# GiantAI/pixtrack

Measured on AMD Instinct MI355X. Metric: tracked frames/sec at 640x480 (full NeRF render + UNet + LM loop), higher is better.
Workload: dtype fp16 storage / fp32 accumulate (UNet, NeRF MLPs); fp32 (LM)

## Files before the change

include/pixtrack_hip.h:

```cpp
#ifndef PIXTRACK_HIP_H
#define PIXTRACK_HIP_H

#include <stdint.h>

#ifdef __cplusplus
extern "C" {
#endif

#define PXT_OK 0
#define PXT_E_ARG -1
#define PXT_E_HIP -2
#define PXT_E_TIMEOUT -3
#define PXT_E_STATE -4

#define PXT_MAX_LEVELS 8
#define PXT_LM_LOG_STRIDE 20

int pxt_version(void);
const char* pxt_last_error(void);
int pxt_device_cus(int* n_cus_host);

typedef struct {
  const float* fmap;
  const float* fref;
// ... 133 lines not shown
  int32_t width, height, spp;
  int32_t mode;
} pxt_ngp_view;

int pxt_ngp_render(pxt_ngp* ctx, const pxt_ngp_view* view_host, float* out_rgba,
                   uint64_t* stats ,
                   void* stream);

int pxt_ngp_render_both(pxt_ngp* ctx, const pxt_ngp_view* view_host, float* out_rgba, float* out_depth_rgba,
                        uint64_t* stats, void* stream);

int pxt_ngp_render_both_from_pose(pxt_ngp* ctx, const pxt_ngp_view* view_host, const float* pose12,
                                  const double* conv27_host, float* cam_out13, float* out_rgba,
                                  float* out_depth_rgba, uint64_t* stats, void* stream);

typedef struct {
  float* rgba;
  float* depth_rgba;
  uint8_t* rgb_u8;
  uint8_t* depth_nz;
} pxt_ngp_outputs;
int pxt_ngp_render_frame(pxt_ngp* ctx, const pxt_ngp_view* view_host, int32_t mode, int32_t camera_from_slot,
                         const pxt_ngp_outputs* out, uint64_t* stats, void* stream);
float* pxt_ngp_camera_slot(pxt_ngp* ctx);

#define PXT_NGP_MAX_BATCH 16
int64_t pxt_ngp_batch_workspace_bytes(int32_t n_renders);
int pxt_ngp_render_frame_batch(pxt_ngp* const* ctxs, const pxt_ngp_view* views_host, int32_t n_renders,
                               const int32_t* modes, int32_t camera_from_slot, const pxt_ngp_outputs* outs_host,
                               uint64_t* const* stats, void* batch_workspace, void* stream);

int pxt_ngp_create_shared(pxt_ngp* src, pxt_ngp** out_ctx);

int pxt_ngp_timing_enable(pxt_ngp* ctx, int32_t every_nth);
int pxt_ngp_timing_read(pxt_ngp* ctx, float* total_ms_host, int32_t* n_launches_host);

int pxt_ngp_query(pxt_ngp* ctx, const float* pos, const float* dir, int32_t n, float* out, void* stream);

int pxt_depth_mask(const float* depth_rgba, int32_t H, int32_t W, int32_t n_erode,
                   int32_t n_dilate, uint8_t* mask_out, uint8_t* tmp, void* stream);
int pxt_depth_mask_plane(const uint8_t* depth_nz, int32_t H, int32_t W, int32_t n_erode, int32_t n_dilate,
                         uint8_t* mask_out, uint8_t* tmp, void* stream);
int pxt_rgba_to_u8(const float* rgba, int32_t H, int32_t W, float alpha_thresh, uint8_t* rgb_out,
                   void* stream);
int pxt_resize_linear(const float* src, int32_t H, int32_t W, int32_t C, float* dst, int32_t Ho,
                      int32_t Wo, void* stream);

int pxt_resize_activity(const uint8_t* mask, const uint8_t* image_u8, int32_t H, int32_t W, int32_t Ho, int32_t Wo,
                        uint8_t* active_out, void* stream);

#ifdef __cplusplus
}
#endif
#endif
```

pixtrack_amd/_lib.py:

```python
from __future__ import annotations

import ctypes as C
import os
from pathlib import Path
from typing import Optional

import torch

_HERE = Path(__file__).resolve().parent
LIB_PATH = Path(os.environ["PIXTRACK_HIP_LIB"]) if os.environ.get("PIXTRACK_HIP_LIB") else _HERE / "libpixtrack_hip.so"

PXT_MAX_LEVELS = 8
PXT_LM_LOG_STRIDE = 20
PXT_E_TIMEOUT = -3
ABI_VERSION = 12
PXT_LM_MAX_BATCH = 16
PXT_UNET_MAX_BATCH = 16
PXT_NGP_MAX_BATCH = 16


class PxtError(RuntimeError):
    """Infrastructure failure of the native path (never a tracking failure)."""


class LmLevel(C.Structure):
    _fields_ = [
        ("fmap", C.c_void_p),
        ("fref", C.c_void_p),
        ("h", C.c_int32),
        ("w", C.c_int32),
        ("C", C.c_int32),
        ("cstride", C.c_int32),
        ("cam", C.c_float * 10),
        ("ndist", C.c_int32),
        ("lambda_", C.c_float * 6),
    ]


class LmConf(C.Structure):
    _fields_ = [
        ("num_iters", C.c_int32),
        ("pad", C.c_int32),
        ("loss", C.c_int32),
        ("loss_alpha", C.c_float),
        ("loss_scale", C.c_float),
        ("grad_stop", C.c_float),
        ("dt_stop", C.c_float),
        ("dR_stop", C.c_float),
# ... 90 lines not shown
    "pxt_unet_workspace_bytes": (_I64, [_VP, _I32, _I32]),
    "pxt_unet_forward": (
        C.c_int,
        [_VP, _VP, _I32, _VP, _I32, _I32, C.POINTER(_VP), C.POINTER(_I32), _I32, _VP, _VP],
    ),
    "pxt_unet_set_defer_join": (C.c_int, [_VP, _I32]),
    "pxt_unet_set_batch_plan": (C.c_int, [_VP, _I32]),
    "pxt_unet_set_tile_skip": (C.c_int, [_VP, _I32]),
    "pxt_unet_pair_join": (C.c_int, [_VP, _VP]),
    "pxt_unet_activation_stats": (C.c_int, [_VP, _I32, _I32, _VP, _VP, _VP]),
    "pxt_unet_workspace_bytes_batch": (_I64, [_VP, _I32, _I32, _I32]),
    "pxt_unet_forward_batch": (
        C.c_int,
        [_VP, _I32, C.POINTER(_VP), C.POINTER(_I32), C.POINTER(_VP), _I32, _I32, C.POINTER(_VP), C.POINTER(_I32),
         C.POINTER(_I32), _VP, _VP],
    ),
    "pxt_unet_workspace_bytes_pair": (_I64, [_VP, C.POINTER(_I32), C.POINTER(_I32)]),
    "pxt_unet_forward_pair": (
        C.c_int,
        [_VP, C.POINTER(_VP), C.POINTER(_I32), C.POINTER(_VP), C.POINTER(_I32), C.POINTER(_I32), C.POINTER(_VP),
         C.POINTER(_I32), C.POINTER(_I32), _VP, _VP],
    ),
    "pxt_conv3x3_nhwc_f16": (C.c_int, [_VP, _I32, _I32, _I32, _VP, _VP, _I32, _I32, _VP, _VP]),
    "pxt_conv3x3_packed_bytes": (_I64, [_I32, _I32]),
    "pxt_conv3x3_pack_weights": (C.c_int, [_VP, _I32, _I32, _VP, _VP]),
    "pxt_conv3x3_packed": (C.c_int, [_VP, _I32, _I32, _I32, _VP, _VP, _I32, _I32, _VP, _VP, _I32, _I32, _VP, _I64, _VP]),
    "pxt_ngp_create": (C.c_int, [C.POINTER(NgpModel), _VP, _I64, _VP, _I64, _VP, _I64, C.POINTER(_VP)]),
    "pxt_ngp_destroy": (C.c_int, [_VP]),
    "pxt_ngp_render": (C.c_int, [_VP, C.POINTER(NgpView), _VP, _VP, _VP]),
    "pxt_ngp_render_both": (C.c_int, [_VP, C.POINTER(NgpView), _VP, _VP, _VP, _VP]),
    "pxt_ngp_render_both_from_pose": (C.c_int, [_VP, C.POINTER(NgpView), _VP, C.POINTER(C.c_double), _VP, _VP, _VP, _VP, _VP]),
    "pxt_ngp_render_frame": (C.c_int, [_VP, C.POINTER(NgpView), _I32, _I32, C.POINTER(NgpOutputs), _VP, _VP]),
    "pxt_ngp_camera_slot": (_VP, [_VP]),
    "pxt_ngp_batch_workspace_bytes": (_I64, [_I32]),
    "pxt_ngp_render_frame_batch": (C.c_int, [C.POINTER(_VP), C.POINTER(NgpView), _I32, C.POINTER(_I32), _I32,
                                              C.POINTER(NgpOutputs), C.POINTER(_VP), _VP, _VP]),
    "pxt_ngp_create_shared": (C.c_int, [_VP, C.POINTER(_VP)]),
    "pxt_ngp_timing_enable": (C.c_int, [_VP, _I32]),
    "pxt_ngp_timing_read": (C.c_int, [_VP, C.POINTER(C.c_float), C.POINTER(_I32)]),
    "pxt_ngp_query": (C.c_int, [_VP, _VP, _VP, _I32, _VP, _VP]),
    "pxt_depth_mask": (C.c_int, [_VP, _I32, _I32, _I32, _I32, _VP, _VP, _VP]),
    "pxt_depth_mask_plane": (C.c_int, [_VP, _I32, _I32, _I32, _I32, _VP, _VP, _VP]),
    "pxt_rgba_to_u8": (C.c_int, [_VP, _I32, _I32, C.c_float, _VP, _VP]),
    "pxt_resize_linear": (C.c_int, [_VP, _I32, _I32, _I32, _VP, _I32, _I32, _VP]),
    "pxt_resize_activity": (C.c_int, [_VP, _VP, _I32, _I32, _I32, _I32, _VP, _VP]),
}


def lib() -> C.CDLL:
    global _lib
    if _lib is not None:
        return _lib
    if not LIB_PATH.exists():
        raise PxtError(
            f"{LIB_PATH} not built. Run `python -m pixtrack_amd._build` (hipcc, gfx950). "
            "There is no CPU fallback for the product path."
        )
    L = C.CDLL(str(LIB_PATH), mode=os.RTLD_NOW | os.RTLD_LOCAL)
    missing = []
    for name, (res, args) in PROTOTYPES.items():
        try:
            fn = getattr(L, name)
        except AttributeError:
            missing.append(name)
            continue
        fn.restype = res
# ... 35 lines not shown
```

pixtrack_amd/csrc/pxt_core.hip:

```cpp
#include "pxt_common.h"

#include <cstdio>
#include <cstring>
#include <mutex>

namespace pxt {
static thread_local char g_last_error[512] = "";
void set_last_error(const char* what, hipError_t e) {
  snprintf(g_last_error, sizeof(g_last_error), "%s: %s", what, hipGetErrorString(e));
}

hipStream_t shared_side_stream(int i) {
  static std::mutex mu;
  static hipStream_t pool[16][3] = {};
  int dev = 0;
  if (hipGetDevice(&dev) != hipSuccess || dev < 0 || dev >= 16 || i < 0 || i > 2) return nullptr;
  std::lock_guard<std::mutex> lock(mu);
  if (!pool[dev][i] && hipStreamCreateWithFlags(&pool[dev][i], hipStreamNonBlocking) != hipSuccess) pool[dev][i] = nullptr;
  return pool[dev][i];
}
}

extern "C" int pxt_version(void) { return 12; }
extern "C" const char* pxt_last_error(void) { return pxt::g_last_error; }
extern "C" int pxt_device_cus(int* n_cus) {
  if (!n_cus) return PXT_E_ARG;
  int dev = 0;
  PXT_HIP_CHECK(hipGetDevice(&dev));
  hipDeviceProp_t prop;
  PXT_HIP_CHECK(hipGetDeviceProperties(&prop, dev));
  *n_cus = prop.multiProcessorCount;
  return PXT_OK;
}
```

pixtrack_amd/csrc/pxt_ngp.hip:

```cpp
#include "pxt_common.h"

#include <algorithm>
#include <atomic>
#include <cmath>
#include <cstdlib>
#include <cstring>
#include <utility>
#include <vector>

namespace pxt {

typedef _Float16 half_t;
typedef __attribute__((ext_vector_type(8))) _Float16 half8;
typedef __attribute__((ext_vector_type(2))) _Float16 half2_t;
typedef __attribute__((ext_vector_type(16))) float f32x16;
typedef __attribute__((ext_vector_type(4))) unsigned u32x4;

constexpr int kGrid = 128;
constexpr int kMaxLevels = 16;
constexpr int kNumFrags = 24;
constexpr int kFragD1 = 0, kFragD2 = 4, kFragC1 = 8, kFragC2 = 12, kFragC3 = 20;

struct NgpLevel {
  float scale;
  unsigned res, offset, size, hashed;
};

struct NgpParams {
  const unsigned* grid;
  unsigned grid_bytes;
  const half8* wfrag;
  const uint8_t* occ;
  NgpLevel lv[kMaxLevels];
  int n_levels, cascades;
  float aabb_scale, cone_angle, depth_scale, dt_lo, dt_hi;
  float cam[12];
  const float* cam_dev;
  float focal, k1;
  float lo[3], hi[3];
  float bg[4];
  float min_T;
  int W, H, spp, mode;
  int coop;
  int srgb_to_linear;
  float* out;
  float* out_depth;
  uint8_t* out_u8;
  uint8_t* out_nz;
  unsigned long long* stats;
};

__device__ inline float calc_dt(float t, float cone, float lo, float hi) {
  return fminf(fmaxf(t * cone, lo), hi);
}

__device__ inline int frexp_exp(float v) {
  const unsigned b = __builtin_bit_cast(unsigned, v);
  const int e = (int)((b >> 23) & 0xffu);
  return e == 0 ? 0 : e - 126;
}

__device__ inline float pow2i(int k) { return __builtin_bit_cast(float, (unsigned)(127 + k) << 23); }
// ... 74 lines not shown
#pragma unroll
  for (int c = 0; c < 8; ++c) {
    float w = 1.0f;
    w = w * ((c & 1) ? ax : (1.0f - ax));
    w = w * ((c & 2) ? ay : (1.0f - ay));
    w = w * ((c & 4) ? az : (1.0f - az));
    const half2_t hv = __builtin_bit_cast(half2_t, vals[c]);
    f0 += w * (float)hv[0];
    f1 += w * (float)hv[1];
  }
  return pack_h2(f0, f1);
}

typedef __attribute__((ext_vector_type(2))) unsigned uint2_t;
typedef __attribute__((ext_vector_type(2))) float float2_t;
__device__ __forceinline__ unsigned ngp_trilinear_pk(const unsigned (&vals)[8], float ax, float ay, float az) {
#pragma clang fp contract(fast)
  const float2_t wx = {1.0f - ax, ax};
  const float wy0 = 1.0f - ay, wz0 = 1.0f - az;
  const float2_t wxy[2] = {wx * wy0, wx * ay};
  float2_t f = {0.f, 0.f};
#pragma unroll
  for (int c = 0; c < 8; c += 2) {
    const float2_t w = wxy[(c >> 1) & 1] * ((c & 4) ? az : wz0);
#pragma unroll
    for (int x = 0; x < 2; ++x) {
      const half2_t hv = __builtin_bit_cast(half2_t, vals[c + x]);
      const float2_t v = {(float)hv[0], (float)hv[1]};
      f += w[x] * v;
    }
  }
  return pack_h2(f[0], f[1]);
}
__device__ inline unsigned ngp_encode_level_uniform(const __amdgpu_buffer_rsrc_t grid, const NgpLevel& Lv, float ux,
                                                    float uy, float uz) {
#pragma clang fp contract(fast)
  const float qx = ux * Lv.scale + 0.5f, qy = uy * Lv.scale + 0.5f, qz = uz * Lv.scale + 0.5f;
  const float fx = floorf(qx), fy = floorf(qy), fz = floorf(qz);
  const float ax = qx - fx, ay = qy - fy, az = qz - fz;
  const unsigned gx = (unsigned)(int)fx, gy = (unsigned)(int)fy, gz = (unsigned)(int)fz;
  unsigned vals[8];
  const int base = (int)(Lv.offset * 4u);
  const unsigned gx4[2] = {gx << 2, (gx << 2) + 4u};
  if (Lv.hashed) {
    const unsigned mask4 = (Lv.size - 1u) << 2;
    const unsigned hy[2] = {gy * (2654435761u * 4u), gy * (2654435761u * 4u) + 2654435761u * 4u};
    const unsigned hz[2] = {gz * (805459861u * 4u), gz * (805459861u * 4u) + 805459861u * 4u};
#pragma unroll
    for (int c = 0; c < 8; ++c) {
      const unsigned off = (gx4[c & 1] ^ hy[(c >> 1) & 1] ^ hz[(c >> 2) & 1]) & mask4;
      vals[c] = (unsigned)__builtin_amdgcn_raw_buffer_load_b32(grid, (int)off, base, 0);
    }
  } else {
    const unsigned r4 = Lv.res * 4u, r24 = Lv.res * Lv.res * 4u, last4 = (Lv.size - 1u) << 2;
    const unsigned ry[2] = {gy * r4, gy * r4 + r4};
    const unsigned rz[2] = {gz * r24, gz * r24 + r24};
#pragma unroll
    for (int c = 0; c < 8; ++c) {
      const unsigned off = min(gx4[c & 1] + ry[(c >> 1) & 1] + rz[(c >> 2) & 1], last4);
      vals[c] = (unsigned)__builtin_amdgcn_raw_buffer_load_b32(grid, (int)off, base, 0);
    }
  }
  return ngp_trilinear_pk(vals, ax, ay, az);
}

template <bool DEPTH_ONLY>
__device__ inline void ngp_mlp_block(const half8* s_w, int lane, half8 x0, half8 x1, half8 shb, float& logit,
                                     float* rgb) {
  f32x16 h1[2];
#pragma unroll
  for (int rb = 0; rb < 2; ++rb) {
    f32x16 a = {0};
    a = __builtin_amdgcn_mfma_f32_32x32x16_f16(s_w[(kFragD1 + 2 * rb) * 64 + lane], x0, a, 0, 0, 0);
    a = __builtin_amdgcn_mfma_f32_32x32x16_f16(s_w[(kFragD1 + 2 * rb + 1) * 64 + lane], x1, a, 0, 0, 0);
    h1[rb] = a;
  }
  f32x16 dout = {0};
#pragma unroll
  for (int q = 0; q < 4; ++q)
    dout = __builtin_amdgcn_mfma_f32_32x32x16_f16(s_w[(kFragD2 + q) * 64 + lane],
                                                  relu_pack8(h1[q >> 1], 8 * (q & 1), true), dout, 0, 0, 0);
  logit = dout[0];
  if (DEPTH_ONLY) {
    rgb[0] = rgb[1] = rgb[2] = 0.f;
    return;
  }
  f32x16 c1[2];
#pragma unroll
  for (int rb = 0; rb < 2; ++rb) {
    f32x16 a = {0};
    a = __builtin_amdgcn_mfma_f32_32x32x16_f16(s_w[(kFragC1 + 2 * rb) * 64 + lane], relu_pack8(dout, 0, false), a,
                                               0, 0, 0);
    a = __builtin_amdgcn_mfma_f32_32x32x16_f16(s_w[(kFragC1 + 2 * rb + 1) * 64 + lane], shb, a, 0, 0, 0);
    c1[rb] = a;
  }
  half8 c1p[4];
// ... 23 lines not shown
#pragma unroll
  for (int i = 0; i < 8; ++i) swap32(Flo[i], Fhi[i]);
  float l0, l1, c0[3], c1[3];
  ngp_mlp_block<DEPTH_ONLY>(s_w, lane, as_half8(Flo[0], Flo[1], Flo[2], Flo[3]), as_half8(Flo[4], Flo[5], Flo[6], Flo[7]),
                            as_half8(shB0[0], shB0[1], shB0[2], shB0[3]), l0, c0);
  __builtin_amdgcn_sched_barrier(0);
  ngp_mlp_block<DEPTH_ONLY>(s_w, lane, as_half8(Fhi[0], Fhi[1], Fhi[2], Fhi[3]), as_half8(Fhi[4], Fhi[5], Fhi[6], Fhi[7]),
                            as_half8(shB1[0], shB1[1], shB1[2], shB1[3]), l1, c1);
  unsigned r0 = __builtin_bit_cast(unsigned, fmaxf(l0, -1e30f)), r1 = __builtin_bit_cast(unsigned, fmaxf(l1, -1e30f));
  swap32(r0, r1);
  logit = __builtin_bit_cast(float, r0);
#pragma unroll
  for (int c = 0; c < 3; ++c) {
    unsigned a0 = __builtin_bit_cast(unsigned, c0[c]), a1 = __builtin_bit_cast(unsigned, c1[c]);
    swap32(a0, a1);
    rgbv[c] = __builtin_bit_cast(float, a0);
  }
}

template <bool DEPTH_ONLY>
__device__ inline void ngp_eval(const NgpParams& P, const half8* s_w, int lane, bool alive, float ux,
                                float uy, float uz, const unsigned* shB0, const unsigned* shB1,
                                float& logit, float* rgbv) {
  unsigned Flo[8], Fhi[8];
#pragma unroll
  for (int l = 0; l < kMaxLevels; ++l) {
    unsigned pk = 0u;
    if (alive && l < P.n_levels) pk = ngp_encode_level(P.grid, P.lv[l], ux, uy, uz);
    if (l < 8) Flo[l] = pk; else Fhi[l - 8] = pk;
  }
  ngp_mlp<DEPTH_ONLY>(s_w, lane, Flo, Fhi, shB0, shB1, logit, rgbv);
}

constexpr int kK = 8;
constexpr int kCtrWords = 16;


struct Ray {
  float o[3], d[3], idir[3];
  float tmin, tmax, zdot;
  bool hit;
};

__device__ inline void ray_clip(const NgpParams& P, Ray& r) {
  const float half_s = P.aabb_scale * 0.5f;
  r.tmin = -INFINITY;
  r.tmax = INFINITY;
#pragma unroll
  for (int a = 0; a < 3; ++a) {
    const float lo = fmaxf(P.lo[a], 0.5f - half_s), hi = fminf(P.hi[a], 0.5f + half_s);
    const float t0 = (lo - r.o[a]) * r.idir[a], t1 = (hi - r.o[a]) * r.idir[a];
    r.tmin = fmaxf(r.tmin, fminf(t0, t1));
    r.tmax = fminf(r.tmax, fmaxf(t0, t1));
  }
  r.hit = r.tmax > fmaxf(r.tmin, 0.f);
}

__device__ __forceinline__ const float* camera_pointer(const NgpParams& P) {
  const float* c = P.cam_dev ? P.cam_dev : P.cam;
  asm volatile("" : "+v"(c));
  return c;
}
__device__ inline void load_camera(const NgpParams& P, float* cam) {
  const float* c = camera_pointer(P);
#pragma unroll
  for (int i = 0; i < 12; ++i) cam[i] = c[i];
// ... 186 lines not shown
      if (lane >= m) inc += o;
    }
    if (lane == 63) s_wave[wave] = inc;
    __syncthreads();
    int wave_off = 0, tile_total = 0;
#pragma unroll
    for (int w = 0; w < 4; ++w) {
      if (w < wave) wave_off += s_wave[w];
      tile_total += s_wave[w];
    }
    if (threadIdx.x == 0) s_base = tile_total ? atomicAdd(Wk.counters, tile_total) : 0;
    __syncthreads();
    int dst = s_base + wave_off + inc - cnt;
    const float4 rdir = make_float4(r.d[0], r.d[1], r.d[2], r.zdot);
#pragma unroll
    for (int j = 0; j < 8; ++j) {
      if (!k[j]) continue;
      Wk.rid[dst] = rid_new[j];
      Wk.t0[dst] = t_start[j];
      if (P.spp == 8) {
        Wk.dir[dst] = rdir;
      } else {
        const int pix = (int)(rid_new[j] / (unsigned)P.spp);
        const Ray rr = make_ray(P, pix % P.W, pix / P.W);
        Wk.dir[dst] = make_float4(rr.d[0], rr.d[1], rr.d[2], rr.zdot);
      }
      ++dst;
    }
    __syncthreads();
  }
}

__device__ __forceinline__ void ngp_march_group(const NgpParams& P, const Ray& r, bool alive, float& t, float4& sp,
                                                float& sample_t, bool& exhausted) {
  const int lane = threadIdx.x & 63, j = lane & 7;
  int k = 0, have = 0;
  bool out = false, busy = alive;
  float pending = -INFINITY;
  float ts = 0.f;
  while (__any(busy)) {
    if (busy) {
      float tt[9];
      tt[0] = t;
#pragma unroll
      for (int i = 0; i < 8; ++i) tt[i + 1] = tt[i] + calc_dt(tt[i], P.cone_angle, P.dt_lo, P.dt_hi);
      float tj = tt[0];
      unsigned ge_tmax = 0u;
#pragma unroll
      for (int i = 0; i < 8; ++i) {
        tj = (j == i) ? tt[i] : tj;
        ge_tmax |= (tt[i] >= r.tmax ? 1u : 0u) << i;
      }
      bool occ = false;
      float target = -INFINITY;
      if (tj < r.tmax && tj >= pending) {
        float pos[3], dt;
        int mip;
        occ = probe_cell(P, r, tj, pos, dt, mip);
        if (!occ) target = cell_exit_t(r, tj, pos, mip);
      }
      int nxt = 8;
#pragma unroll
      for (int i = 7; i >= 1; --i) nxt = (i > j && tt[i] >= target) ? i : nxt;
      unsigned word = (occ ? 8u : (unsigned)(nxt - 1)) << (4 * j);
      word |= __shfl_xor(word, 1, 8);
      word |= __shfl_xor(word, 2, 8);
      word |= __shfl_xor(word, 4, 8);
      if (__all(!busy || (k == 0 && word == 0x88888888u && ge_tmax == 0u && pending == -INFINITY))) {
        if (busy) {
          ts = tj;
          have = 1;
          k = kK;
          t = tt[8];
          busy = false;
        }
        continue;
      }
      int cur = 8;
#pragma unroll
      for (int i = 7; i >= 0; --i) cur = (tt[i] >= pending) ? i : cur;
      int last_skip = -1, mine = -1;
      while (cur < 8 && k < kK) {
        if ((ge_tmax >> cur) & 1u) { out = true; break; }
        const unsigned nb = (word >> (4 * cur)) & 15u;
        if (nb & 8u) {
          if (k == j) mine = cur;
          ++k; ++cur; last_skip = -1;
        } else {
          last_skip = cur;
          cur = (int)(nb & 7u) + 1;
        }
      }
      float t_cur = tt[8];
#pragma unroll
      for (int i = 0; i < 8; ++i) {
        t_cur = (cur == i) ? tt[i] : t_cur;
        if (mine == i) { ts = tt[i]; have = 1; }
      }
      const float tg = __shfl(target, (lane & ~7) | (last_skip >= 0 ? last_skip : j), 64);
      if (last_skip >= 0) pending = (tt[8] < tg) ? tg : -INFINITY;
      else if (!(pending > tt[8])) pending = -INFINITY;
      t = t_cur;
      busy = !out && k < kK;
    }
  }
  sp = make_float4(0.f, 0.f, 0.f, 0.f);
  sample_t = 0.f;
  if (have) {
    sp.x = r.o[0] + ts * r.d[0]; sp.y = r.o[1] + ts * r.d[1]; sp.z = r.o[2] + ts * r.d[2];
    sp.w = calc_dt(ts, P.cone_angle, P.dt_lo, P.dt_hi);
// ... 22 lines not shown
}

__device__ __forceinline__ int ngp_patch_point_offset(const NgpLevel& Lv, int lane, unsigned lox, unsigned loy, unsigned loz) {
  const unsigned lx = lox + (unsigned)(lane & 3), ly = loy + (unsigned)((lane >> 2) & 3), lz = loz + (unsigned)(lane >> 4);
  unsigned idx;
  if (Lv.hashed) idx = (lx ^ (ly * 2654435761u) ^ (lz * 805459861u)) & (Lv.size - 1u);
  else idx = min(lx + ly * Lv.res + lz * Lv.res * Lv.res, Lv.size - 1u);
  return (int)(idx << 2);
}
__device__ __forceinline__ unsigned ngp_encode_level_patch(const unsigned* patch, const NgpLevel& Lv, float ux, float uy, float uz,
                                                           unsigned lox, unsigned loy, unsigned loz, bool in_box) {
#pragma clang fp contract(fast)
  const float qx = ux * Lv.scale + 0.5f, qy = uy * Lv.scale + 0.5f, qz = uz * Lv.scale + 0.5f;
  const float fx = floorf(qx), fy = floorf(qy), fz = floorf(qz);
  const float ax = qx - fx, ay = qy - fy, az = qz - fz;
  const unsigned gx = (unsigned)(int)fx, gy = (unsigned)(int)fy, gz = (unsigned)(int)fz;
  const unsigned local = in_box ? (gx - lox) + 4u * (gy - loy) + 16u * (gz - loz) : 0u;
  const unsigned* c0 = patch + local;
  const unsigned vals[8] = {c0[0], c0[1], c0[4], c0[5], c0[16], c0[17], c0[20], c0[21]};
  return ngp_trilinear_pk(vals, ax, ay, az);
}

template <int MODE>
__device__ __forceinline__ void ngp_render_body(const NgpParams& P, const NgpWork& Wk, int rays_per_wg, int blk, int nblk,
                                                half8* s_w, unsigned* s_feat, float* s_rays) {
  const int n = Wk.counters[0];
  if (P.stats && blk == 0 && threadIdx.x == 0) atomicAdd(P.stats + 1, (unsigned long long)n);
  const int knee = min(nblk, 4096);
  const int by_div = (n + rays_per_wg - 1) / rays_per_wg;
  const int by_div2 = (int)(((long long)n * 16) / ((long long)rays_per_wg * 21));
  const int n_wg = min(nblk, max(knee / 4, max(min(by_div, knee), by_div2)));
  if (blk >= n_wg || blk * 32 >= n) return;
  for (int i = threadIdx.x; i < kNumFrags * 64; i += 256) s_w[i] = P.wfrag[i];
  const __amdgpu_buffer_rsrc_t grid_rsrc = __builtin_amdgcn_make_buffer_rsrc((void*)P.grid, 0, (int)P.grid_bytes, 0x00020000);
  const float enc_lo = 0.5f - P.aabb_scale * 0.5f, enc_inv = 1.0f / P.aabb_scale;
  __syncthreads();
  const int lane = threadIdx.x & 63, wave = threadIdx.x >> 6;
  const int rlane = lane >> 3, k = lane & 7;
  unsigned long long n_samples = 0;
  int n_steps = 0, n_box_levels = 0;
  const int n_waves = n_wg * 4, wave_id = blk * 4 + wave;
  auto stream_slot = [&](int s) { return ((s >> 3) * n_waves + wave_id) * 8 + (s & 7); };
  int cursor = 8;
  int slot = stream_slot(rlane);
  bool alive = slot < n;
  float* const s_ray = s_rays + (wave * 8 + rlane) * 8;
  float t = 0.f;
  float4 rd = make_float4(0.f, 0.f, 1.f, 0.f);
  if (alive) {
    t = Wk.t0[slot];
    rd = Wk.dir[slot];
  }
  if (k == 0) {
    s_ray[0] = 1.f;
    s_ray[1] = s_ray[2] = s_ray[3] = s_ray[4] = s_ray[5] = 0.f;
    s_ray[6] = __builtin_bit_cast(float, alive ? Wk.rid[slot] : 0u);
  }
  unsigned* const col = s_feat + wave * (8 * 64) + lane;
  const int tl = ((lane & 7) << 3) | (lane >> 3);
  unsigned* const wcol = s_feat + wave * (8 * 64) + tl;
  while (__any(alive)) {
    float4 sp;
    float sample_t;
    bool exhausted;
    {
      const Ray r = ray_from_record(P, rd);
      ngp_march_group(P, r, alive, t, sp, sample_t, exhausted);
    }
    const float dt = alive ? sp.w : 0.f;
    const bool valid = dt != 0.f;
    unsigned Flo[8] = {0u, 0u, 0u, 0u, 0u, 0u, 0u, 0u}, Fhi[8] = {0u, 0u, 0u, 0u, 0u, 0u, 0u, 0u};
    float logit = 0.f, rgbv[3] = {0.f, 0.f, 0.f};
    if (__any(valid)) {
      float ux = (sp.x - enc_lo) * enc_inv, uy = (sp.y - enc_lo) * enc_inv, uz = (sp.z - enc_lo) * enc_inv;
      ux = __shfl(ux, tl, 64); uy = __shfl(uy, tl, 64); uz = __shfl(uz, tl, 64);
      const unsigned long long vmask = __ballot(valid);
      const bool valid_t = (vmask >> tl) & 1ull;
      ++n_steps;
      float coop_scale = 0.f;
      float emin[3] = {0.f, 0.f, 0.f};
      if (P.coop) {
        const int first = __ffsll((long long)vmask) - 1;
        const float d0[3] = {__builtin_bit_cast(float, __builtin_amdgcn_readlane(__builtin_bit_cast(int, rd.x), first)),
                             __builtin_bit_cast(float, __builtin_amdgcn_readlane(__builtin_bit_cast(int, rd.y), first)),
                             __builtin_bit_cast(float, __builtin_amdgcn_readlane(__builtin_bit_cast(int, rd.z), first))};
        if (__all(!valid || (rd.x == d0[0] && rd.y == d0[1] && rd.z == d0[2]))) {
          const float tlo = wave_minmax<false>(valid ? sample_t : INFINITY), thi = wave_minmax<true>(valid ? sample_t : -INFINITY);
          float ext = 0.f;
#pragma unroll
          for (int a = 0; a < 3; ++a) {
            const float o = camera_pointer(P)[4 * a + 3];
            const float ea = ((o + tlo * d0[a]) - enc_lo) * enc_inv, eb = ((o + thi * d0[a]) - enc_lo) * enc_inv;
            emin[a] = __builtin_bit_cast(float, __builtin_amdgcn_readfirstlane(__builtin_bit_cast(int, fminf(ea, eb))));
            ext = fmaxf(ext, fabsf(eb - ea));
          }
          coop_scale = __builtin_bit_cast(float, __builtin_amdgcn_readfirstlane(__builtin_bit_cast(int, 1.98f / ext)));
        }
      }
#pragma unroll
      for (int half = 0; half < 2; ++half) {
        const int l0 = 8 * half;
        int n_coop = 0;
        if (P.coop) {
          asm volatile("s_waitcnt lgkmcnt(0)" ::: "memory");
          while (n_coop < 8 && P.lv[l0 + n_coop].scale <= coop_scale) {
            const NgpLevel& Lv = P.lv[l0 + n_coop];
            unsigned lo[3];
            {
#pragma clang fp contract(fast)
              lo[0] = (unsigned)(int)floorf(emin[0] * Lv.scale + 0.5f);
              lo[1] = (unsigned)(int)floorf(emin[1] * Lv.scale + 0.5f);
              lo[2] = (unsigned)(int)floorf(emin[2] * Lv.scale + 0.5f);
            }
            __builtin_amdgcn_raw_ptr_buffer_load_lds(grid_rsrc, (__attribute__((address_space(3))) void*)(s_feat + wave * (8 * 64) + n_coop * 64),
                                                     4, ngp_patch_point_offset(Lv, lane, lo[0], lo[1], lo[2]), (int)(Lv.offset * 4u), 0, 0);
            ++n_coop;
          }
          n_box_levels += n_coop;
        }
#pragma unroll 4
        for (int l = n_coop; l < 8; ++l) wcol[l * 64] = ngp_encode_level_uniform(grid_rsrc, P.lv[l0 + l], ux, uy, uz);
        if (n_coop) {
          asm volatile("s_waitcnt vmcnt(0)" ::: "memory");
          __builtin_amdgcn_wave_barrier();
          for (int l = 0; l < n_coop; ++l) {
            const NgpLevel& Lv = P.lv[l0 + l];
            unsigned lo[3];
            {
#pragma clang fp contract(fast)
              lo[0] = (unsigned)(int)floorf(emin[0] * Lv.scale + 0.5f);
              lo[1] = (unsigned)(int)floorf(emin[1] * Lv.scale + 0.5f);
              lo[2] = (unsigned)(int)floorf(emin[2] * Lv.scale + 0.5f);
            }
            const unsigned pk = ngp_encode_level_patch(s_feat + wave * (8 * 64) + l * 64, Lv, ux, uy, uz, lo[0], lo[1], lo[2], valid_t);
            __builtin_amdgcn_wave_barrier();
            wcol[l * 64] = pk;
          }
        }
        __builtin_amdgcn_wave_barrier();
        if (half == 0) {
#pragma unroll
          for (int l = 0; l < 8; ++l) Flo[l] = valid ? col[l * 64] : 0u;
        } else {
#pragma unroll
          for (int l = 0; l < 8; ++l) Fhi[l] = valid ? col[l * 64] : 0u;
        }
        __builtin_amdgcn_wave_barrier();
      }
// ... 32 lines not shown
      ca += __shfl_xor(ca, m, 8);
      if (MODE == 2) cd += __shfl_xor(cd, m, 8);
    }
    if (contributes) n_samples += 1;
    const unsigned long long vb = __ballot(valid);
    const unsigned vgrp = (unsigned)((vb >> (rlane * 8)) & 0xFFull);
    const int n_valid = __popc(vgrp);
    const int k_last = grp ? k_term : n_valid - 1;
    const float T_new = (k_last >= 0) ? __shfl(T_after, rlane * 8 + max(k_last, 0), 64) : T0;
    if (alive) {
      const bool terminated = grp != 0;
      const bool closes = terminated || exhausted;
      if (k == 0) {
        float4 acc = make_float4(s_ray[1] + cr, s_ray[2] + cg, s_ray[3] + cb, s_ray[4] + ca);
        float accd = 0.f;
        if (MODE == 2) accd = s_ray[5] + cd;
        if (closes) {
          const unsigned rid = __builtin_bit_cast(unsigned, s_ray[6]);
          if (MODE == 2) Wk.sppbuf_d[rid] = terminated ? accd / acc.w : accd;
          if (terminated) {
            acc.x /= acc.w; acc.y /= acc.w; acc.z /= acc.w; acc.w = 1.0f;
          }
          Wk.sppbuf[rid] = acc;
        } else {
          s_ray[0] = T_new;
          s_ray[1] = acc.x; s_ray[2] = acc.y; s_ray[3] = acc.z; s_ray[4] = acc.w;
          if (MODE == 2) s_ray[5] = accd;
        }
      }
      if (closes) alive = false;
    }
    const unsigned long long dead = __ballot(!alive && k == 0);
    if (dead) {
      const int rank = __popcll(dead & ((1ull << (rlane * 8)) - 1ull));
      if (!alive) {
        const int ns = stream_slot(cursor + rank);
        if (ns < n) {
          alive = true;
          t = Wk.t0[ns];
          rd = Wk.dir[ns];
          if (k == 0) {
            s_ray[0] = 1.f;
            s_ray[1] = s_ray[2] = s_ray[3] = s_ray[4] = s_ray[5] = 0.f;
            s_ray[6] = __builtin_bit_cast(float, Wk.rid[ns]);
          }
        }
      }
      cursor += __popcll(dead);
    }
  }
  if (P.stats) {
    __shared__ unsigned long long s_cnt[4][3];
    for (int m = 32; m >= 1; m >>= 1) n_samples += __shfl_xor(n_samples, m, 64);
    if (lane == 0) {
      s_cnt[wave][0] = n_samples;
      s_cnt[wave][1] = (unsigned long long)n_steps;
      s_cnt[wave][2] = (unsigned long long)n_box_levels;
    }
    __syncthreads();
    if (threadIdx.x < 3) {
      const unsigned long long tot = s_cnt[0][threadIdx.x] + s_cnt[1][threadIdx.x] + s_cnt[2][threadIdx.x] + s_cnt[3][threadIdx.x];
      if (tot) atomicAdd(P.stats + (threadIdx.x == 0 ? 0 : threadIdx.x + 1), tot);
    }
  }
}

__global__ void ngp_pose_to_camera_kernel(const float* __restrict__ pose12, const PoseConv cv, float* __restrict__ cam_dev,
                                          float* __restrict__ cam_out) {
  if (threadIdx.x != 0 || blockIdx.x != 0) return;
  float cam[12];
  pose_to_camera_f64(pose12, cv, cam);
  for (int i = 0; i < 12; ++i) {
    cam_dev[i] = cam[i];
    if (cam_out) cam_out[i] = cam[i];
  }
  if (cam_out) __hip_atomic_store(&cam_out[12], 1.f, __ATOMIC_RELEASE, __HIP_MEMORY_SCOPE_SYSTEM);
}

__device__ inline float srgb_to_linear(float c) {
  if (c <= 0.04045f) return c / 12.92f;
  return __builtin_amdgcn_exp2f(2.4f * __builtin_amdgcn_logf((c + 0.055f) / 1.055f));
}

// ... 80 lines not shown
__global__ __launch_bounds__(256) void ngp_raygen_kernel_m(const NgpBatchItem* __restrict__ items) {
  const NgpBatchItem& it = items[blockIdx.y];
  ngp_raygen_body(it.P, it.W, blockIdx.x, gridDim.x);
}

template <int MODES>
__device__ __forceinline__ void ngp_render_impl(const NgpBatchItem& it, int rays_per_wg) {
  __shared__ half8 s_w[kNumFrags * 64];
  __shared__ unsigned s_feat[4 * 8 * 64];
  __shared__ float s_rays[4 * 8 * 8];
  const int mode = MODES == 3 ? it.P.mode : MODES;
  if (mode == 0) ngp_render_body<0>(it.P, it.W, rays_per_wg, blockIdx.x, gridDim.x, s_w, s_feat, s_rays);
  else if (mode == 1) ngp_render_body<1>(it.P, it.W, rays_per_wg, blockIdx.x, gridDim.x, s_w, s_feat, s_rays);
  else ngp_render_body<2>(it.P, it.W, rays_per_wg, blockIdx.x, gridDim.x, s_w, s_feat, s_rays);
}
template <int MODES>
__global__ __launch_bounds__(256) __attribute__((amdgpu_waves_per_eu(4, 4))) void ngp_render_kernel_v(const NgpItemsByValue<4> items,
                                                                                                   int rays_per_wg) {
  ngp_render_impl<MODES>(ngp_kernarg_item(blockIdx.y), rays_per_wg);
}
template <int MODES>
__global__ __launch_bounds__(256) __attribute__((amdgpu_waves_per_eu(4, 4))) void ngp_render_kernel_m(
    const NgpBatchItem* __restrict__ items, int rays_per_wg) {
  ngp_render_impl<MODES>(items[blockIdx.y], rays_per_wg);
}

__global__ __launch_bounds__(256) void ngp_resolve_kernel_v(const NgpItemsByValue<4> items) {
  const NgpBatchItem& it = ngp_kernarg_item(blockIdx.y);
  ngp_resolve_body(it.P, it.W, blockIdx.x);
}
__global__ __launch_bounds__(256) void ngp_resolve_kernel_m(const NgpBatchItem* __restrict__ items) {
  const NgpBatchItem& it = items[blockIdx.y];
  ngp_resolve_body(it.P, it.W, blockIdx.x);
}

__global__ __launch_bounds__(256) void ngp_query_kernel(const NgpParams P, const float* __restrict__ pos,
                                                        const float* __restrict__ dir, int n,
                                                        float* __restrict__ out) {
  __shared__ half8 s_w[kNumFrags * 64];
  for (int i = threadIdx.x; i < kNumFrags * 64; i += 256) s_w[i] = P.wfrag[i];
  __syncthreads();
  const int lane = threadIdx.x & 63;
  const int i = blockIdx.x * 256 + threadIdx.x;
  const bool ok = i < n;
  const int ii = ok ? i : 0;
  const float half_s = P.aabb_scale * 0.5f;
  const float scene_lo = 0.5f - half_s, inv_s = 1.0f / P.aabb_scale;
  float sh[16];
  sh4_eval(dir[3 * ii], dir[3 * ii + 1], dir[3 * ii + 2], sh);
  unsigned shB0[4], shB1[4];
#pragma unroll
  for (int k = 0; k < 4; ++k) {
    shB0[k] = pack_h2(sh[2 * k], sh[2 * k + 1]);
    shB1[k] = pack_h2(sh[8 + 2 * k], sh[8 + 2 * k + 1]);
    swap32(shB0[k], shB1[k]);
  }
  float logit, rgbv[3];
  ngp_eval<false>(P, s_w, lane, ok, (pos[3 * ii] - scene_lo) * inv_s, (pos[3 * ii + 1] - scene_lo) * inv_s,
           (pos[3 * ii + 2] - scene_lo) * inv_s, shB0, shB1, logit, rgbv);
  if (ok) {
    out[4 * i] = logit;
    out[4 * i + 1] = rgbv[0];
    out[4 * i + 2] = rgbv[1];
    out[4 * i + 3] = rgbv[2];
  }
}

}

struct NgpTables {
  unsigned* grid = nullptr;
  unsigned grid_bytes = 0;
  pxt::half8* wfrag = nullptr;
  uint8_t* occ = nullptr;
  std::atomic<int> refs{1};
};

struct pxt_ngp {
  pxt_ngp_model model;
  NgpTables* tab = nullptr;
  float* cam_dev = nullptr;
  pxt::NgpLevel lv[pxt::kMaxLevels];
  void* scratch = nullptr;
  size_t scratch_rays = 0;
  bool counters_clean = false;
  pxt::NgpWork work;
  int timing = 0;
  long long renders = 0;
  std::vector<std::pair<hipEvent_t, hipEvent_t>> events;
  std::vector<std::pair<hipEvent_t, hipEvent_t>> pool;
};

using namespace pxt;

namespace {

int kappa(int kind, int q, int h, int j) {
  if (kind == 0) return 16 * h + 8 * q + j;
  if (kind == 1) return 32 * (q >> 1) + 16 * (q & 1) + 8 * (j >> 2) + 4 * h + (j & 3);
  if (q == 0) return 8 * (j >> 2) + 4 * h + (j & 3);
  return 16 + 8 * h + j;
}

void pack_layer(const uint16_t* W, int n_out, int n_in, int kind, int frag0, std::vector<uint16_t>& dst) {
  const int n_rb = (n_out + 31) / 32, n_q = n_in / 16;
  for (int rb = 0; rb < n_rb; ++rb)
    for (int q = 0; q < n_q; ++q)
      for (int lane = 0; lane < 64; ++lane)
        for (int j = 0; j < 8; ++j) {
          const int row = 32 * rb + (lane & 31), h = lane >> 5;
          const int col = kappa(kind, q, h, j);
          const uint16_t v = (row < n_out) ? W[(size_t)row * n_in + col] : (uint16_t)0;
          dst[((size_t)(frag0 + rb * n_q + q) * 64 + lane) * 8 + j] = v;
        }
}

void release_tables(NgpTables* t) {
  if (!t || --t->refs > 0) return;
  if (t->grid) (void)hipFree(t->grid);
  if (t->wfrag) (void)hipFree(t->wfrag);
  if (t->occ) (void)hipFree(t->occ);
  delete t;
}

int init_camera_slot(pxt_ngp* ctx) {
  const float cam0[16] = {1.f, 0.f, 0.f, 0.5f, 0.f, 1.f, 0.f, 0.5f, 0.f, 0.f, 1.f, -1.f, 0.f, 0.f, 0.f, 0.f};
  hipError_t e = hipMalloc((void**)&ctx->cam_dev, sizeof(cam0));
  if (e == hipSuccess) e = hipMemcpy(ctx->cam_dev, cam0, sizeof(cam0), hipMemcpyHostToDevice);
  if (e != hipSuccess) { set_last_error("pxt_ngp camera slot", e); return PXT_E_HIP; }
  return PXT_OK;
}

}

extern "C" int pxt_ngp_create(const pxt_ngp_model* model, const void* grid_params, int64_t n_grid_params,
                              const void* mlp_params, int64_t n_mlp_params, const uint8_t* occupancy,
                              int64_t n_occ_bytes, pxt_ngp** out_ctx) {
  if (!model || !grid_params || !mlp_params || !occupancy || !out_ctx) return PXT_E_ARG;
  if (model->n_levels < 1 || model->n_levels > kMaxLevels || model->n_features != 2) return PXT_E_ARG;
  if (model->n_levels != 16) return PXT_E_ARG;
  if (model->grid_cascades < 1 || model->grid_cascades > 8) return PXT_E_ARG;
  if (n_mlp_params != 64 * 32 + 16 * 64 + 64 * 32 + 64 * 64 + 16 * 64) return PXT_E_ARG;
  if (n_occ_bytes != (int64_t)model->grid_cascades * kGrid * kGrid * kGrid / 8) return PXT_E_ARG;
  pxt_ngp* ctx = new pxt_ngp();
  ctx->model = *model;
  const unsigned Tsz = 1u << model->log2_hashmap;
  unsigned off = 0;
  for (int l = 0; l < model->n_levels; ++l) {
    const double scale = std::exp2((double)l * std::log2((double)model->per_level_scale)) * model->base_res - 1.0;
    const unsigned res = (unsigned)std::ceil(scale) + 1;
    unsigned long long n = (unsigned long long)res * res * res;
    unsigned sz = n > Tsz ? Tsz : (unsigned)n;
    sz = (sz + 7) / 8 * 8;
    sz = sz < Tsz ? sz : Tsz;
    ctx->lv[l].scale = (float)scale;
    ctx->lv[l].res = res;
    ctx->lv[l].offset = off;
    ctx->lv[l].size = sz;
    ctx->lv[l].hashed = n > sz ? 1u : 0u;
    off += sz;
  }
  if (n_grid_params != (int64_t)off * 2) { delete ctx; return PXT_E_ARG; }
  std::vector<uint16_t> frag((size_t)kNumFrags * 64 * 8);
  const uint16_t* mp = (const uint16_t*)mlp_params;
  pack_layer(mp, 64, 32, 0, kFragD1, frag);
  pack_layer(mp + 2048, 16, 64, 1, kFragD2, frag);
  pack_layer(mp + 3072, 64, 32, 2, kFragC1, frag);
  pack_layer(mp + 5120, 64, 64, 1, kFragC2, frag);
  pack_layer(mp + 9216, 16, 64, 1, kFragC3, frag);
  NgpTables* t = ctx->tab = new NgpTables();
  t->grid_bytes = (unsigned)((size_t)off * 4);
  hipError_t e = hipMalloc((void**)&t->grid, (size_t)off * 4);
  if (e == hipSuccess) e = hipMalloc((void**)&t->wfrag, frag.size() * 2);
  if (e == hipSuccess) e = hipMalloc((void**)&t->occ, (size_t)n_occ_bytes);
  if (e == hipSuccess) e = hipMemcpy(t->grid, grid_params, (size_t)off * 4, hipMemcpyHostToDevice);
  if (e == hipSuccess) e = hipMemcpy(t->wfrag, frag.data(), frag.size() * 2, hipMemcpyHostToDevice);
  if (e == hipSuccess) e = hipMemcpy(t->occ, occupancy, (size_t)n_occ_bytes, hipMemcpyHostToDevice);
  if (e != hipSuccess) {
    set_last_error("pxt_ngp_create", e);
    pxt_ngp_destroy(ctx);
    return PXT_E_HIP;
  }
  if (const int rc = init_camera_slot(ctx)) { pxt_ngp_destroy(ctx); return rc; }
  *out_ctx = ctx;
  return PXT_OK;
}

extern "C" int pxt_ngp_create_shared(pxt_ngp* src, pxt_ngp** out_ctx) {
  if (!src || !src->tab || !out_ctx) return PXT_E_ARG;
  pxt_ngp* ctx = new pxt_ngp();
  ctx->model = src->model;
  for (int l = 0; l < kMaxLevels; ++l) ctx->lv[l] = src->lv[l];
  ctx->tab = src->tab;
  ++ctx->tab->refs;
  if (const int rc = init_camera_slot(ctx)) { pxt_ngp_destroy(ctx); return rc; }
  *out_ctx = ctx;
  return PXT_OK;
}

extern "C" int pxt_ngp_destroy(pxt_ngp* ctx) {
  if (!ctx) return PXT_E_ARG;
  release_tables(ctx->tab);
  if (ctx->cam_dev) (void)hipFree(ctx->cam_dev);
  if (ctx->scratch) (void)hipFree(ctx->scratch);
  for (auto& ev : ctx->events) { (void)hipEventDestroy(ev.first); (void)hipEventDestroy(ev.second); }
  for (auto& ev : ctx->pool) { (void)hipEventDestroy(ev.first); (void)hipEventDestroy(ev.second); }
  delete ctx;
  return PXT_OK;
}

static void fill_model(const pxt_ngp* ctx, NgpParams& P) {
  std::memset(&P, 0, sizeof(P));
  P.grid = ctx->tab->grid;
  P.grid_bytes = ctx->tab->grid_bytes;
  P.wfrag = ctx->tab->wfrag;
  P.occ = ctx->tab->occ;
  for (int l = 0; l < kMaxLevels; ++l) P.lv[l] = ctx->lv[l < ctx->model.n_levels ? l : 0];
  P.n_levels = ctx->model.n_levels;
  P.cascades = ctx->model.grid_cascades;
  P.aabb_scale = ctx->model.aabb_scale;
  P.cone_angle = ctx->model.cone_angle;
  P.depth_scale = ctx->model.depth_scale;
  P.srgb_to_linear = ctx->model.linear_colors ? 0 : 1;
  static const int coop_rt = [] { const char* e = getenv("PXT_NGP_COOP"); return e ? atoi(e) : 1; }();
  P.coop = coop_rt;
  P.dt_lo = (float)(std::sqrt(3.0) / 1024.0);
  P.dt_hi = P.dt_lo * (float)(1 << (P.cascades - 1)) * (float)(1024 / kGrid);
}

extern "C" int pxt_ngp_query(pxt_ngp* ctx, const float* pos, const float* dir, int32_t n, float* out,
                             void* stream) {
  if (!ctx || !pos || !dir || !out || n < 1) return PXT_E_ARG;
  NgpParams P;
  fill_model(ctx, P);
  hipLaunchKernelGGL(ngp_query_kernel, dim3((n + 255) / 256), dim3(256), 0, (hipStream_t)stream, P, pos, dir, n,
                     out);
  PXT_HIP_CHECK(hipGetLastError());
  return PXT_OK;
}

static int ensure_scratch(pxt_ngp* ctx, size_t rays) {
  if (ctx->scratch && ctx->scratch_rays >= rays) return PXT_OK;
  const size_t cap = rays + 2 * kTile;
  if (ctx->scratch) {
    hipError_t e0 = hipDeviceSynchronize();
    (void)e0;
// ... 262 lines not shown
```

Baseline: 710.5.

## Store hash grid in fp32 alongside fp16 and gather fp32 corners

At model creation, the fp16 hash-grid table is expanded into an fp32 copy held in the same allocation, with the original fp16 data placed after it. The per-level encoder then does 64-bit buffer loads of float2 corners and interpolates in plain fp32 instead of unpacking half2 values. The cooperative LDS patch path keeps reading the fp16 region through a base offset. This aims to remove the conversion and packed-math work in the interpolation, at the cost of doubling gather bandwidth and cache footprint for the grid. Diagnostic counters guarded by a compile flag are also added.

```diff
diff --git a/include/pixtrack_hip.h b/include/pixtrack_hip.h
--- a/include/pixtrack_hip.h
+++ b/include/pixtrack_hip.h
@@ -189,6 +189,8 @@
 
 int pxt_ngp_create_shared(pxt_ngp* src, pxt_ngp** out_ctx);
 
+const float* pxt_ngp_grid_f32(pxt_ngp* ctx);
+
 int pxt_ngp_timing_enable(pxt_ngp* ctx, int32_t every_nth);
 int pxt_ngp_timing_read(pxt_ngp* ctx, float* total_ms_host, int32_t* n_launches_host);
 
diff --git a/pixtrack_amd/_lib.py b/pixtrack_amd/_lib.py
--- a/pixtrack_amd/_lib.py
+++ b/pixtrack_amd/_lib.py
@@ -13,7 +13,7 @@
 PXT_MAX_LEVELS = 8
 PXT_LM_LOG_STRIDE = 20
 PXT_E_TIMEOUT = -3
-ABI_VERSION = 12
+ABI_VERSION = 13
 PXT_LM_MAX_BATCH = 16
 PXT_UNET_MAX_BATCH = 16
 PXT_NGP_MAX_BATCH = 16
@@ -170,6 +170,7 @@
     "pxt_ngp_render_both_from_pose": (C.c_int, [_VP, C.POINTER(NgpView), _VP, C.POINTER(C.c_double), _VP, _VP, _VP, _VP, _VP]),
     "pxt_ngp_render_frame": (C.c_int, [_VP, C.POINTER(NgpView), _I32, _I32, C.POINTER(NgpOutputs), _VP, _VP]),
     "pxt_ngp_camera_slot": (_VP, [_VP]),
+    "pxt_ngp_grid_f32": (_VP, [_VP]),
     "pxt_ngp_batch_workspace_bytes": (_I64, [_I32]),
     "pxt_ngp_render_frame_batch": (C.c_int, [C.POINTER(_VP), C.POINTER(NgpView), _I32, C.POINTER(_I32), _I32,
                                               C.POINTER(NgpOutputs), C.POINTER(_VP), _VP, _VP]),
diff --git a/pixtrack_amd/csrc/pxt_core.hip b/pixtrack_amd/csrc/pxt_core.hip
--- a/pixtrack_amd/csrc/pxt_core.hip
+++ b/pixtrack_amd/csrc/pxt_core.hip
@@ -21,7 +21,7 @@
 }
 }
 
-extern "C" int pxt_version(void) { return 12; }
+extern "C" int pxt_version(void) { return 13; }
 extern "C" const char* pxt_last_error(void) { return pxt::g_last_error; }
 extern "C" int pxt_device_cus(int* n_cus) {
   if (!n_cus) return PXT_E_ARG;
diff --git a/pixtrack_amd/csrc/pxt_ngp.hip b/pixtrack_amd/csrc/pxt_ngp.hip
--- a/pixtrack_amd/csrc/pxt_ngp.hip
+++ b/pixtrack_amd/csrc/pxt_ngp.hip
@@ -28,6 +28,7 @@
 
 struct NgpParams {
   const unsigned* grid;
+  const float* grid32;
   unsigned grid_bytes;
   const half8* wfrag;
   const uint8_t* occ;
@@ -168,36 +169,50 @@
   }
   return pack_h2(f[0], f[1]);
 }
-__device__ inline unsigned ngp_encode_level_uniform(const __amdgpu_buffer_rsrc_t grid, const NgpLevel& Lv, float ux,
+__device__ __forceinline__ unsigned ngp_trilinear_f32(const float2_t (&vals)[8], float ax, float ay, float az) {
+#pragma clang fp contract(fast)
+  const float2_t wx = {1.0f - ax, ax};
+  const float wy0 = 1.0f - ay, wz0 = 1.0f - az;
+  const float2_t wxy[2] = {wx * wy0, wx * ay};
+  float2_t f = {0.f, 0.f};
+#pragma unroll
+  for (int c = 0; c < 8; c += 2) {
+    const float2_t w = wxy[(c >> 1) & 1] * ((c & 4) ? az : wz0);
+#pragma unroll
+    for (int x = 0; x < 2; ++x) f += w[x] * vals[c + x];
+  }
+  return pack_h2(f[0], f[1]);
+}
+__device__ inline unsigned ngp_encode_level_uniform(const __amdgpu_buffer_rsrc_t grid32, const NgpLevel& Lv, float ux,
                                                     float uy, float uz) {
 #pragma clang fp contract(fast)
   const float qx = ux * Lv.scale + 0.5f, qy = uy * Lv.scale + 0.5f, qz = uz * Lv.scale + 0.5f;
   const float fx = floorf(qx), fy = floorf(qy), fz = floorf(qz);
   const float ax = qx - fx, ay = qy - fy, az = qz - fz;
   const unsigned gx = (unsigned)(int)fx, gy = (unsigned)(int)fy, gz = (unsigned)(int)fz;
-  unsigned vals[8];
-  const int base = (int)(Lv.offset * 4u);
-  const unsigned gx4[2] = {gx << 2, (gx << 2) + 4u};
+  float2_t vals[8];
+  const int base = (int)(Lv.offset * 8u);
+  const unsigned gx8[2] = {gx << 3, (gx << 3) + 8u};
   if (Lv.hashed) {
-    const unsigned mask4 = (Lv.size - 1u) << 2;
-    const unsigned hy[2] = {gy * (2654435761u * 4u), gy * (2654435761u * 4u) + 2654435761u * 4u};
-    const unsigned hz[2] = {gz * (805459861u * 4u), gz * (805459861u * 4u) + 805459861u * 4u};
+    const unsigned mask8 = (Lv.size - 1u) << 3;
+    const unsigned hy[2] = {gy * (2654435761u * 8u), gy * (2654435761u * 8u) + 2654435761u * 8u};
+    const unsigned hz[2] = {gz * (805459861u * 8u), gz * (805459861u * 8u) + 805459861u * 8u};
 #pragma unroll
     for (int c = 0; c < 8; ++c) {
-      const unsigned off = (gx4[c & 1] ^ hy[(c >> 1) & 1] ^ hz[(c >> 2) & 1]) & mask4;
-      vals[c] = (unsigned)__builtin_amdgcn_raw_buffer_load_b32(grid, (int)off, base, 0);
+      const unsigned off = (gx8[c & 1] ^ hy[(c >> 1) & 1] ^ hz[(c >> 2) & 1]) & mask8;
+      vals[c] = __builtin_bit_cast(float2_t, __builtin_amdgcn_raw_buffer_load_b64(grid32, (int)off, base, 0));
     }
   } else {
-    const unsigned r4 = Lv.res * 4u, r24 = Lv.res * Lv.res * 4u, last4 = (Lv.size - 1u) << 2;
-    const unsigned ry[2] = {gy * r4, gy * r4 + r4};
-    const unsigned rz[2] = {gz * r24, gz * r24 + r24};
+    const unsigned r8 = Lv.res * 8u, r28 = Lv.res * Lv.res * 8u, last8 = (Lv.size - 1u) << 3;
+    const unsigned ry[2] = {gy * r8, gy * r8 + r8};
+    const unsigned rz[2] = {gz * r28, gz * r28 + r28};
 #pragma unroll
     for (int c = 0; c < 8; ++c) {
-      const unsigned off = min(gx4[c & 1] + ry[(c >> 1) & 1] + rz[(c >> 2) & 1], last4);
-      vals[c] = (unsigned)__builtin_amdgcn_raw_buffer_load_b32(grid, (int)off, base, 0);
-    }
-  }
-  return ngp_trilinear_pk(vals, ax, ay, az);
+      const unsigned off = min(gx8[c & 1] + ry[(c >> 1) & 1] + rz[(c >> 2) & 1], last8);
+      vals[c] = __builtin_bit_cast(float2_t, __builtin_amdgcn_raw_buffer_load_b64(grid32, (int)off, base, 0));
+    }
+  }
+  return ngp_trilinear_f32(vals, ax, ay, az);
 }
 
 template <bool DEPTH_ONLY>
@@ -287,6 +302,12 @@
   ngp_mlp<DEPTH_ONLY>(s_w, lane, Flo, Fhi, shB0, shB1, logit, rgbv);
 }
 
+#if PXT_EXP_STAMPS
+__device__ unsigned long long g_ngp_diag[4];
+#define PXT_DIAG_COUNT(var) (++(var))
+#else
+#define PXT_DIAG_COUNT(var) ((void)0)
+#endif
 constexpr int kK = 8;
 constexpr int kCtrWords = 16;
 
@@ -539,13 +560,14 @@
 }
 
 __device__ __forceinline__ void ngp_march_group(const NgpParams& P, const Ray& r, bool alive, float& t, float4& sp,
-                                                float& sample_t, bool& exhausted) {
+                                                float& sample_t, bool& exhausted, int& n_trips, int& n_walks) {
   const int lane = threadIdx.x & 63, j = lane & 7;
   int k = 0, have = 0;
   bool out = false, busy = alive;
   float pending = -INFINITY;
   float ts = 0.f;
   while (__any(busy)) {
+    PXT_DIAG_COUNT(n_trips);
     if (busy) {
       float tt[9];
       tt[0] = t;
@@ -583,6 +605,7 @@
         }
         continue;
       }
+      PXT_DIAG_COUNT(n_walks);
       int cur = 8;
 #pragma unroll
       for (int i = 7; i >= 0; --i) cur = (tt[i] >= pending) ? i : cur;
@@ -671,13 +694,16 @@
   const int n_wg = min(nblk, max(knee / 4, max(min(by_div, knee), by_div2)));
   if (blk >= n_wg || blk * 32 >= n) return;
   for (int i = threadIdx.x; i < kNumFrags * 64; i += 256) s_w[i] = P.wfrag[i];
-  const __amdgpu_buffer_rsrc_t grid_rsrc = __builtin_amdgcn_make_buffer_rsrc((void*)P.grid, 0, (int)P.grid_bytes, 0x00020000);
+  const __amdgpu_buffer_rsrc_t grid_rsrc = __builtin_amdgcn_make_buffer_rsrc((void*)P.grid32, 0, (int)(3u * P.grid_bytes), 0x00020000);
+  const int f16_base = (int)(2u * P.grid_bytes);
   const float enc_lo = 0.5f - P.aabb_scale * 0.5f, enc_inv = 1.0f / P.aabb_scale;
   __syncthreads();
   const int lane = threadIdx.x & 63, wave = threadIdx.x >> 6;
   const int rlane = lane >> 3, k = lane & 7;
   unsigned long long n_samples = 0;
   int n_steps = 0, n_box_levels = 0;
+  int n_trips = 0, n_walks = 0, n_refills = 0;
+  (void)n_trips; (void)n_walks; (void)n_refills;
   const int n_waves = n_wg * 4, wave_id = blk * 4 + wave;
   auto stream_slot = [&](int s) { return ((s >> 3) * n_waves + wave_id) * 8 + (s & 7); };
   int cursor = 8;
@@ -704,7 +730,7 @@
     bool exhausted;
     {
       const Ray r = ray_from_record(P, rd);
-      ngp_march_group(P, r, alive, t, sp, sample_t, exhausted);
+      ngp_march_group(P, r, alive, t, sp, sample_t, exhausted, n_trips, n_walks);
     }
     const float dt = alive ? sp.w : 0.f;
     const bool valid = dt != 0.f;
@@ -752,7 +778,7 @@
               lo[2] = (unsigned)(int)floorf(emin[2] * Lv.scale + 0.5f);
             }
             __builtin_amdgcn_raw_ptr_buffer_load_lds(grid_rsrc, (__attribute__((address_space(3))) void*)(s_feat + wave * (8 * 64) + n_coop * 64),
-                                                     4, ngp_patch_point_offset(Lv, lane, lo[0], lo[1], lo[2]), (int)(Lv.offset * 4u), 0, 0);
+                                                     4, ngp_patch_point_offset(Lv, lane, lo[0], lo[1], lo[2]), f16_base + (int)(Lv.offset * 4u), 0, 0);
             ++n_coop;
           }
           n_box_levels += n_coop;
@@ -851,6 +877,9 @@
     }
     const unsigned long long dead = __ballot(!alive && k == 0);
     if (dead) {
+#if PXT_EXP_STAMPS
+      if (__any(!alive && stream_slot(cursor + __popcll(dead & ((1ull << (rlane * 8)) - 1ull))) < n)) ++n_refills;
+#endif
       const int rank = __popcll(dead & ((1ull << (rlane * 8)) - 1ull));
       if (!alive) {
         const int ns = stream_slot(cursor + rank);
@@ -868,6 +897,13 @@
       cursor += __popcll(dead);
     }
   }
+#if PXT_EXP_STAMPS
+  if (lane == 0) {
+    atomicAdd(&g_ngp_diag[0], (unsigned long long)n_trips);
+    atomicAdd(&g_ngp_diag[1], (unsigned long long)n_walks);
+    atomicAdd(&g_ngp_diag[2], (unsigned long long)n_refills);
+  }
+#endif
   if (P.stats) {
     __shared__ unsigned long long s_cnt[4][3];
     for (int m = 32; m >= 1; m >>= 1) n_samples += __shfl_xor(n_samples, m, 64);
@@ -1014,6 +1050,13 @@
 __global__ __launch_bounds__(256) void ngp_resolve_kernel_m(const NgpBatchItem* __restrict__ items) {
   const NgpBatchItem& it = items[blockIdx.y];
   ngp_resolve_body(it.P, it.W, blockIdx.x);
+}
+
+__global__ __launch_bounds__(256) void ngp_grid_to_f32_kernel(const unsigned* __restrict__ grid, float2* __restrict__ out, unsigned n) {
+  for (unsigned i = blockIdx.x * 256u + threadIdx.x; i < n; i += gridDim.x * 256u) {
+    const half2_t h = __builtin_bit_cast(half2_t, grid[i]);
+    out[i] = make_float2((float)h[0], (float)h[1]);
+  }
 }
 
 __global__ __launch_bounds__(256) void ngp_query_kernel(const NgpParams P, const float* __restrict__ pos,
@@ -1052,6 +1095,7 @@
 
 struct NgpTables {
   unsigned* grid = nullptr;
+  float* grid32 = nullptr;
   unsigned grid_bytes = 0;
   pxt::half8* wfrag = nullptr;
   uint8_t* occ = nullptr;
@@ -1099,7 +1143,7 @@
 
 void release_tables(NgpTables* t) {
   if (!t || --t->refs > 0) return;
-  if (t->grid) (void)hipFree(t->grid);
+  if (t->grid32) (void)hipFree(t->grid32);
   if (t->wfrag) (void)hipFree(t->wfrag);
   if (t->occ) (void)hipFree(t->occ);
   delete t;
@@ -1152,12 +1196,18 @@
   pack_layer(mp + 9216, 16, 64, 1, kFragC3, frag);
   NgpTables* t = ctx->tab = new NgpTables();
   t->grid_bytes = (unsigned)((size_t)off * 4);
-  hipError_t e = hipMalloc((void**)&t->grid, (size_t)off * 4);
+  hipError_t e = hipMalloc((void**)&t->grid32, (size_t)off * 12);
+  if (e == hipSuccess) t->grid = (unsigned*)(t->grid32 + (size_t)off * 2);
   if (e == hipSuccess) e = hipMalloc((void**)&t->wfrag, frag.size() * 2);
   if (e == hipSuccess) e = hipMalloc((void**)&t->occ, (size_t)n_occ_bytes);
   if (e == hipSuccess) e = hipMemcpy(t->grid, grid_params, (size_t)off * 4, hipMemcpyHostToDevice);
   if (e == hipSuccess) e = hipMemcpy(t->wfrag, frag.data(), frag.size() * 2, hipMemcpyHostToDevice);
   if (e == hipSuccess) e = hipMemcpy(t->occ, occupancy, (size_t)n_occ_bytes, hipMemcpyHostToDevice);
+  if (e == hipSuccess) {
+    hipLaunchKernelGGL(ngp_grid_to_f32_kernel, dim3(1024), dim3(256), 0, nullptr, t->grid, (float2*)t->grid32, off);
+    e = hipGetLastError();
+  }
+  if (e == hipSuccess) e = hipStreamSynchronize(nullptr);
   if (e != hipSuccess) {
     set_last_error("pxt_ngp_create", e);
     pxt_ngp_destroy(ctx);
@@ -1180,6 +1230,18 @@
   return PXT_OK;
 }
 
+#if PXT_EXP_STAMPS
+extern "C" int pxt_ngp_diag_read(unsigned long long* out_host) {
+  unsigned long long zero[4] = {0, 0, 0, 0};
+  PXT_HIP_CHECK(hipDeviceSynchronize());
+  PXT_HIP_CHECK(hipMemcpyFromSymbol(out_host, HIP_SYMBOL(g_ngp_diag), sizeof(zero)));
+  PXT_HIP_CHECK(hipMemcpyToSymbol(HIP_SYMBOL(g_ngp_diag), zero, sizeof(zero)));
+  return PXT_OK;
+}
+#endif
+
+extern "C" const float* pxt_ngp_grid_f32(pxt_ngp* ctx) { return ctx && ctx->tab ? ctx->tab->grid32 : nullptr; }
+
 extern "C" int pxt_ngp_destroy(pxt_ngp* ctx) {
   if (!ctx) return PXT_E_ARG;
   release_tables(ctx->tab);
@@ -1194,6 +1256,7 @@
 static void fill_model(const pxt_ngp* ctx, NgpParams& P) {
   std::memset(&P, 0, sizeof(P));
   P.grid = ctx->tab->grid;
+  P.grid32 = ctx->tab->grid32;
   P.grid_bytes = ctx->tab->grid_bytes;
   P.wfrag = ctx->tab->wfrag;
   P.occ = ctx->tab->occ;
```

After: 720.2, median of 6. 1.01x the previous value.
